# pkuyzy/ESC-GNN

Measured on AMD Instinct MI355X. Metric: graphs/sec + edges-aggregated/sec, NestedGIN_eff h=3 bs=128 @1/2/4/8 GPU, higher is better.
Workload: dtype f32; 1 GPU; count_cycle-shaped random regular graphs (n in 10/15/20/30), target=triangles, NestedGIN_eff h=3 layers=4 hidden=256, bs=128 per GPU (configs[1]); global_batch=128, parallelism=dp1 graph-sharded, rccl_ranks=1, ranks=1

## Files before the change

esc-gnn_amd/csrc/common.h:

```cpp
#pragma once
#include <hip/hip_runtime.h>
#include <hip/hip_ext.h>
#include <stdint.h>
#include <stdio.h>
#include <stdarg.h>

#include "../../include/escgnn_hip.h"

namespace esc {

constexpr int WAVE = 64;

#ifndef ESC_NODE_PRIO
#define ESC_NODE_PRIO 2
#endif
#define ESC_PRIO() __builtin_amdgcn_s_setprio(ESC_NODE_PRIO)

void set_error(const char* fmt, ...);

#define ESC_REQUIRE(cond, ...)                    \
  do {                                            \
    if (!(cond)) {                                \
      esc::set_error(__VA_ARGS__);                \
      return ESC_EINVAL;                          \
// ... 9 lines not shown
    }                                                                       \
  } while (0)

inline bool aligned16(const void* p) { return (reinterpret_cast<uintptr_t>(p) & 15) == 0; }
inline int64_t cdiv(int64_t a, int64_t b) { return (a + b - 1) / b; }

bool prof_slot(int kind, hipEvent_t* start, hipEvent_t* stop);
unsigned long long* prof_span_next(int kind);
#define ESC_SPAN_WGS 2048
#define ESC_SPAN_WAVES 8192
#define ESC_SPAN_STRIDE (ESC_SPAN_WGS + ESC_SPAN_WAVES)
bool trace_launch();

void arm_launch_event(hipEvent_t ev);
hipEvent_t take_launch_event();

template <typename... KArgs, typename... Args>
inline void launch(int kind, void (*kernel)(KArgs...), dim3 grid, dim3 block, size_t lds, hipStream_t s,
                   Args... args) {
  hipEvent_t a = nullptr, b = nullptr;
  hipEvent_t done = take_launch_event();
  if (done != nullptr) {
    hipStreamCaptureStatus cap = hipStreamCaptureStatusNone;
    if (hipStreamIsCapturing(s, &cap) != hipSuccess || cap != hipStreamCaptureStatusNone) { arm_launch_event(done); done = nullptr; }
  }
  if (prof_slot(kind, &a, &b)) {
    hipExtLaunchKernelGGL(kernel, grid, block, (unsigned)lds, s, a, b, 0, static_cast<KArgs>(args)...);
    if (done != nullptr) (void)hipEventRecord(done, s);
  } else if (done != nullptr) {
    hipExtLaunchKernelGGL(kernel, grid, block, (unsigned)lds, s, nullptr, done, 0, static_cast<KArgs>(args)...);
// ... 43 lines not shown
int gemm_lds_floor();
void set_gemm_lds_floor(int bytes);
int edge_lds_floor();
int node_lds_floor();
void set_node_lds_floor(int bytes);
void set_edge_lds_floor(int bytes);
int norm_rowblock_cap();
void set_norm_rowblock_cap(int v);
bool bn_bwd_one_launch();
void set_bn_bwd_one_launch(int on);
bool bn_bwd_fold();
void set_bn_bwd_fold(int on);
bool last_block_finalize();
void set_last_block_finalize(int on);
void set_linear_knob(int knob, int value);

__device__ __forceinline__ void store_agent(float2* p, float2 v) {
  const unsigned long long bits = ((unsigned long long)__float_as_uint(v.y) << 32) | __float_as_uint(v.x);
  __hip_atomic_store(reinterpret_cast<unsigned long long*>(p), bits, __ATOMIC_RELAXED, __HIP_MEMORY_SCOPE_AGENT);
}

__device__ __forceinline__ bool grid_last_block(unsigned* counter, unsigned nblocks) {
  __shared__ unsigned s_ticket;
  __builtin_amdgcn_s_waitcnt(0x0F70);
  __syncthreads();
  if (threadIdx.x == 0) s_ticket = __hip_atomic_fetch_add(counter, 1u, __ATOMIC_RELAXED, __HIP_MEMORY_SCOPE_AGENT);
  __syncthreads();
  const bool last = s_ticket == nblocks - 1;
  if (last) {
    __builtin_amdgcn_fence(__ATOMIC_ACQUIRE, "agent");
// ... 87 lines not shown
```

esc-gnn_amd/csrc/engine.hip:

```cpp
#include "common.h"

#include <map>
#include <vector>
#include <cstdlib>

namespace esc {

struct Arena {
  float* base;
  int64_t off;
  float* take(int64_t n) {
    float* p = base ? base + off : nullptr;
    off += (n + 63) & ~63LL;
    return p;
  }
};

struct BnWs { float *mean, *invstd, *scale, *shift, *nglob, *coef; };
struct MlpWs { float *Y0, *Y1; BnWs b0, b1; float* A1 = nullptr; };

struct Layout {
  int64_t N, E, Z, H, L, C0, W;
  float *Zb, *Yz; BnWs zb0, zb1;
  float *A0, *Zemb;
// ... 81 lines not shown
  std::vector<esc_reduce_job>* jobs = nullptr;
  float** slab_cursor = nullptr;
  bool on_edge_stream = false;
  int act = 1;
  const float* l1_target = nullptr;
  int64_t l1_denom = 0;
};

struct LdsFloorGuard {
  explicit LdsFloorGuard(bool on) : on_(on && edge_lds_floor() > 0) { if (on_) set_gemm_lds_floor(edge_lds_floor()); }
  ~LdsFloorGuard() { if (on_) set_gemm_lds_floor(0); }
  bool on_;
};

static constexpr int kNodeLdsFloorBwd = 66 * 1024;
struct NodeFloorGuard {
  explicit NodeFloorGuard(int bytes) : on_(bytes > 0) { if (on_) set_node_lds_floor(bytes); }
  ~NodeFloorGuard() { if (on_) set_node_lds_floor(0); }
  bool on_;
};

static int linear_backward(const Ctx& c, const float* dY, int64_t ld_dy, const float* X, int64_t ld_x, const float* sc,
                           const float* sh, const esc_linear_t& lin, int64_t M, float* dX, int64_t ld_dx, int accumulate) {
  const LdsFloorGuard cap(c.on_edge_stream);
  const int64_t N = lin.out_dim, K = lin.in_dim;
  if (c.jobs == nullptr)
    return esc_linear_bwd_both(dY, ld_dy, X, ld_x, sc, sh, lin.w, K, M, N, K, dX, ld_dx, accumulate, lin.dw, K, lin.db,
                               c.y.slabs, c.s);
  float* slabs = *c.slab_cursor;
  *c.slab_cursor += (esc_linear_bwd_weight_scratch(M, N, K) + 63) & ~63LL;
// ... 13 lines not shown
                              int accumulate, const esc_bn_bwd_next* next) {
  const LdsFloorGuard cap(c.on_edge_stream);
  const int64_t N = lin.out_dim, K = lin.in_dim;
  if (c.jobs == nullptr)
    return esc_linear_bwd_both_bn(dOut, ld_dout, &f, X, ld_x, sc, sh, lin.w, K, M, N, K, dX, ld_dx, accumulate, lin.dw, K, lin.db, c.y.slabs,
                                  nullptr, next, c.s);
  float* slabs = *c.slab_cursor;
  *c.slab_cursor += (esc_linear_bwd_weight_scratch(M, N, K) + 63) & ~63LL;
  c.jobs->emplace_back();
  return esc_linear_bwd_both_bn(dOut, ld_dout, &f, X, ld_x, sc, sh, lin.w, K, M, N, K, dX, ld_dx, accumulate, lin.dw, K, lin.db, slabs,
                                &c.jobs->back(), next, c.s);
}

struct EdgeStream {
  hipStream_t stream = nullptr;
  hipEvent_t z_ready = nullptr, joined = nullptr, lin1_fork = nullptr, lin1_rest = nullptr, e_ready[ESC_MAX_LAYERS] = {}, de_ready[ESC_MAX_LAYERS] = {},
             agg_done[ESC_MAX_LAYERS] = {};
  bool ok = false;
};
static int g_use_edge_stream = 1;
static int current_device() {
  int dev = 0;
  (void)hipGetDevice(&dev);
  return dev;
}
static EdgeStream& edge_stream() {
  static thread_local std::map<int, EdgeStream> per_device;
  static thread_local EdgeStream off;
  if (!g_use_edge_stream) return off;
  EdgeStream& es = per_device[current_device()];
  if (!es.ok && es.stream == nullptr) {
    int least = 0, greatest = 0;
    (void)hipDeviceGetStreamPriorityRange(&least, &greatest);
    bool good = hipStreamCreateWithPriority(&es.stream, hipStreamNonBlocking, least) == hipSuccess;
    good = good && hipEventCreateWithFlags(&es.z_ready, hipEventDisableTiming) == hipSuccess;
    good = good && hipEventCreateWithFlags(&es.joined, hipEventDisableTiming) == hipSuccess;
    good = good && hipEventCreateWithFlags(&es.lin1_fork, hipEventDisableTiming) == hipSuccess;
    good = good && hipEventCreateWithFlags(&es.lin1_rest, hipEventDisableTiming) == hipSuccess;
    for (int l = 0; l < ESC_MAX_LAYERS; ++l) {
      good = good && hipEventCreateWithFlags(&es.e_ready[l], hipEventDisableTiming) == hipSuccess;
      good = good && hipEventCreateWithFlags(&es.de_ready[l], hipEventDisableTiming) == hipSuccess;
      good = good && hipEventCreateWithFlags(&es.agg_done[l], hipEventDisableTiming) == hipSuccess;
    }
    es.ok = good;
  }
  return es;
}
static int64_t g_two_stream_min_edges = 12000;
static EdgeStream& edge_stream_for(int64_t edges) {
  static thread_local EdgeStream off;
  return edges >= g_two_stream_min_edges ? edge_stream() : off;
}
static int chain(hipEvent_t ev, hipStream_t src, hipStream_t waiter) {
  if (hipEventRecord(ev, src) != hipSuccess || hipStreamWaitEvent(waiter, ev, 0) != hipSuccess) {
    set_error("esc_engine: stream event failed");
    return ESC_ELAUNCH;
  }
  return ESC_OK;
}

static int g_plain_events = 0;
struct ArmedEvent {
  ArmedEvent(hipEvent_t ev, bool on) : on_(on && !g_plain_events) { if (on_) arm_launch_event(ev); }
  ~ArmedEvent() { if (on_) (void)take_launch_event(); }
  bool on_;
};
static int chain_armed(hipEvent_t ev, const ArmedEvent& arm, hipStream_t src, hipStream_t waiter) {
  const bool bound = arm.on_ && take_launch_event() == nullptr;
  if ((!bound && hipEventRecord(ev, src) != hipSuccess) || (waiter != nullptr && hipStreamWaitEvent(waiter, ev, 0) != hipSuccess)) {
    set_error("esc_engine: stream event failed");
    return ESC_ELAUNCH;
  }
  return ESC_OK;
}

static Ctx edge_ctx(const Ctx& c, hipStream_t edge) {
  Ctx x = c;
  x.s = edge;
  x.on_edge_stream = true;
// ... 314 lines not shown
  const Layout& y = c.y;
  const int64_t N = y.N, E = y.E, H = y.H, L = y.L, W = y.W;
  ESC_TRY(linear_backward(c, y.dpred, 1, y.Yl, H, y.bl.scale, y.bl.shift, m->lin2, N, y.dAl, H, 0));
  const bool split_lin1 = es.ok && c.jobs != nullptr && L >= 1;
  const esc_bn_bwd_fused fl = bn_fused(y.Yl, H, y.bl, 1);
  const bool fa_l = fuse_node_act(c);
  const MlpWs& wl = y.conv[L > 0 ? L - 1 : 0];
  esc_bn_bwd_next nl{y.bst_part, y.cat + L * H, W, wl.b1.mean, wl.b1.invstd, wl.b1.scale, wl.b1.shift, 1};
  auto lin1_ok = [&](int64_t col0, int64_t ncols, const esc_bn_bwd_next* nx) {
    return esc_linear_bwd_both_bn_ok(y.dAl, H, &fl, y.cat + col0, W, m->lin1.w + col0, W, N, H, ncols, y.dcat + col0, W,
                                     c.jobs ? *c.slab_cursor : y.slabs, nx) != 0;
  };
  const bool fuse_l = kBnBwdApplyInGemm && c.act == 1 && !sync_on(c) && y.bst_part != nullptr &&
                      (split_lin1 ? (lin1_ok(0, L * H, nullptr) && lin1_ok(L * H, H, nullptr)) : lin1_ok(0, W, nullptr));
  int64_t last_slots = 0;
  if (fuse_l)
    ESC_TRY(esc_bn_bwd_coef(y.Yl, H, nullptr, 0, y.dAl, H, N, H, y.bl.mean, y.bl.invstd, m->bn_lin1.gamma, m->bn_lin1.beta, 1, y.bl.coef,
                            m->bn_lin1.dgamma, m->bn_lin1.dbeta, y.bn_scratch, c.s));
  else
    ESC_TRY(bn_backward(c, y.Yl, H, nullptr, 0, y.dAl, H, N, y.bl, m->bn_lin1, y.dAl, H, y.bn_scratch));
  if (split_lin1) {
    const int64_t K0 = L * H;
    auto part = [&](void* stream, int64_t col0, int64_t ncols, float* db, const esc_bn_bwd_next* nx) -> int {
      float* slabs = *c.slab_cursor;
      *c.slab_cursor += (esc_linear_bwd_weight_scratch(N, H, ncols) + 63) & ~63LL;
      c.jobs->emplace_back();
      const bool fa = fa_l;
      if (fuse_l)
        return esc_linear_bwd_both_bn(y.dAl, H, &fl, y.cat + col0, W, fa ? y.cat_scale + col0 : nullptr, fa ? y.cat_shift + col0 : nullptr, m->lin1.w + col0, W,
                                      N, H, ncols, y.dcat + col0, W, 0, m->lin1.dw + col0, W, db, slabs, &c.jobs->back(), nx, stream);
      return esc_linear_bwd_both_deferred(y.dAl, H, y.cat + col0, W, fa ? y.cat_scale + col0 : nullptr, fa ? y.cat_shift + col0 : nullptr, m->lin1.w + col0, W, N, H, ncols,
                                          y.dcat + col0, W, 0, m->lin1.dw + col0, W, db, slabs, &c.jobs->back(), stream);
    };
    ESC_TRY(chain(es.lin1_fork, (hipStream_t)c.s, es.stream));
    {
      const LdsFloorGuard cap(true);
      ESC_TRY(part(es.stream, 0, K0, nullptr, nullptr));
    }
    if (hipEventRecord(es.lin1_rest, es.stream) != hipSuccess) { set_error("esc_engine: stream event failed"); return ESC_ELAUNCH; }
    const bool leave = fuse_l && fa_l && kBnBwdSumsFromDx && lin1_ok(K0, H, &nl) &&
                       mlp_backward_fused(c, m->conv[L - 1].nn, y.conv[L - 1], y.agg[L - 1], L == 1 ? y.C0 : H, N, y.cat + L * H, W, y.dcat + L * H, W,
                                          y.dagg, L == 1 ? y.C0 : H, true);
    ESC_TRY(part(c.s, K0, H, m->lin1.db, leave ? &nl : nullptr));
    if (leave) last_slots = cdiv(N, esc_linear_bwd_bn_block_rows(N, H, H));
  } else if (fuse_l) {
    ESC_TRY(linear_backward_bn(c, y.dAl, H, fl, y.cat, W, fa_l ? y.cat_scale : nullptr, fa_l ? y.cat_shift : nullptr, m->lin1, N, y.dcat, W, 0, nullptr));
  } else {
    ESC_TRY(linear_backward(c, y.dAl, H, y.cat, W, fa_l ? y.cat_scale : nullptr, fa_l ? y.cat_shift : nullptr, m->lin1, N, y.dcat, W, 0));
  }
  Ctx ce = es.ok ? edge_ctx(c, es.stream) : c;
  std::vector<esc_reduce_job> edge_jobs;
  edge_jobs.reserve(ESC_MAX_REDUCE_JOBS);
  if (es.ok && c.jobs) ce.jobs = &edge_jobs;
  std::vector<esc_sum_job> eps_jobs;
// ... 45 lines not shown
      ESC_TRY(esc_slab_reduce_jobs(edge_jobs.data(), (int)edge_jobs.size(), es.stream));
      edge_jobs.clear();
    }
  }
  ESC_TRY(mlp_backward(c, m->xemb, y.xemb, b->x, y.C0, N, y.cat, W, y.dcat, W, nullptr, 0, fuse_node_act(c)));
  Ctx ct = ce;
  ct.on_edge_stream = false;
  ESC_TRY(bn_backward(ce, y.Yz, H, nullptr, 0, y.dZemb, H, E, y.zb1, m->zbn1, y.dZemb, H, ce.y.bn_scratch));
  ESC_TRY(linear_backward(ct, y.dZemb, H, y.A0, H, nullptr, nullptr, m->zlin, E, y.dAz, H, 0));
  ESC_TRY(bn_backward(ce, y.Zb, H, nullptr, 0, y.dAz, H, E, y.zb0, m->zbn0, y.dAz, H, ce.y.bn_scratch));
  ESC_TRY(esc_bag_bwd_table_rows(y.dAz, H, H, b->col_ptr, b->col_row, b->col_val, b->col_col, y.Z, m->z_rows, E,
                                 1, m->dz_table, y.bag_scratch, ce.s));
  mark(PH_NODE_BWD_DONE, c.s);
  mark(PH_EDGE_BWD_DONE, ce.s);
  if (!eps_jobs.empty()) ESC_TRY(esc_reduce_sum_jobs(eps_jobs.data(), (int)eps_jobs.size(), c.s));
  if (c.jobs && !c.jobs->empty()) ESC_TRY(esc_slab_reduce_jobs(c.jobs->data(), (int)c.jobs->size(), c.s));
  if (es.ok) {
    if (hipEventRecord(es.joined, es.stream) != hipSuccess) { set_error("esc_engine: stream event failed"); return ESC_ELAUNCH; }
    Pending local;
    Pending& p = defer ? *defer : local;
    p.open = true; p.join = true; p.stream = (hipStream_t)c.s;
    p.edge_jobs.swap(edge_jobs);
    if (!defer) return finish_pending(p);
  }
  return ESC_OK;
}

static Layout plan_layout_zinc(const esc_zinc_gin_t* m, int64_t N, int64_t E, int64_t Z, int64_t G, float* base, bool train) {
  Layout y{};
  Arena a{base, 0};
// ... 518 lines not shown

}

using namespace esc;

extern "C" {

int esc_engine_set_two_stream_min_edges(int64_t edges) {
  g_two_stream_min_edges = edges < 0 ? 0 : edges;
  return ESC_OK;
}

int esc_engine_set_side_stream(int on) {
  g_use_edge_stream = (on & 2) != 0;
  g_plain_events = (on & 64) != 0;
  return ESC_OK;
}

int esc_engine_phase_times(double* out, int skip) {
  PhaseRing& p = phases();
  for (int i = 0; i < 6; ++i) out[i] = 0.0;
  if (!p.on || p.steps < 2) return 0;
  const int first = p.steps > PhaseRing::RING ? p.steps - PhaseRing::RING + 1 : 0;
  int n = 0;
  for (int sidx = first + skip; sidx < p.steps; ++sidx) {
    hipEvent_t* e = p.ev[sidx % PhaseRing::RING];
    bool ok = true;
    for (int k = 0; k < PH_COUNT; ++k) ok = ok && e[k] != nullptr;
    if (!ok) continue;
    float t[6] = {};
// ... 220 lines not shown
```

esc-gnn_amd/csrc/gemm_dma.h:

```cpp
#pragma once
#include "common.h"

namespace esc {
namespace dma {

typedef float f32x16 __attribute__((ext_vector_type(16)));
typedef int i32x4 __attribute__((ext_vector_type(4)));
using lds_void = __attribute__((address_space(3))) void;

__device__ __forceinline__ i32x4 make_rsrc(const void* p, unsigned bytes) {
  const uint64_t a = reinterpret_cast<uint64_t>(p);
  i32x4 r;
  r[0] = (int)(uint32_t)a; r[1] = (int)(uint32_t)((a >> 32) & 0xffffu); r[2] = (int)bytes; r[3] = 0x00020000;
  return r;
}
__device__ __forceinline__ unsigned lds_addr(const float* p) {
  return (unsigned)(uintptr_t)(lds_void*)const_cast<float*>(p);
}
__device__ __forceinline__ void dma16(i32x4 r, unsigned dst, int voff, int soff) {
  unsigned keep;
  asm volatile(
      "s_mov_b32 %0, m0\n\ts_mov_b32 m0, %3\n\ts_nop 4\n\tbuffer_load_dwordx4 %1, %2, %4 offen lds\n\ts_mov_b32 m0, %0"
      : "=&s"(keep)
      : "v"(voff), "s"(r), "s"(dst), "s"(soff)
// ... 688 lines not shown
template <int BM, int BN, int BK, int WM, int WN, int STAGES, int LW, bool A_RM, bool B_RM, int PRO, bool STATS, bool DB, bool INIT = false>
inline hipError_t launch_gemm(GArgs g, size_t lds_floor, hipStream_t s, int kind = ESC_K_LINEAR) {
  using C_ = Cfg<BM, BN, BK, WM, WN, STAGES, LW, A_RM, B_RM, PRO, STATS, DB>;
  auto kern = gemm_kernel<BM, BN, BK, WM, WN, STAGES, LW, A_RM, B_RM, PRO, STATS, DB, INIT>;
  if (BM < 128 && gemm_lds_floor() == 0 && (size_t)node_lds_floor() > lds_floor) lds_floor = (size_t)node_lds_floor();
  const size_t lds = C_::LDS_BYTES > lds_floor ? C_::LDS_BYTES : lds_floor;
  static size_t raised_to = 64 * 1024;
  hipError_t e = raise_lds(kern, lds, raised_to);
  if (e != hipSuccess) return e;
  finish_args<BM, BN>(g);
  const unsigned nwg = (unsigned)(g.ntile_m * g.ntile_n * splits_of(g));
  esc::launch(BM >= 128 && kind == ESC_K_LINEAR ? ESC_K_GEMM_EDGE : kind, kern, dim3(nwg), dim3(C_::NTHR), lds, s, g);
  return hipSuccess;
}

template <int BM, int BN, int BK, int WM, int WN, int STAGES, int LW, bool PRO, bool BNB = false, bool BSTAT = false>
inline hipError_t launch_dual(DualArgs a, size_t lds_floor, hipStream_t s, int kind = ESC_K_LINEAR, hipStream_t s_dw = nullptr) {
  using CX = Cfg<BM, BN, BK, WM, WN, STAGES, LW, false, true, (BNB ? 4 : 0) | (BSTAT ? 8 : 0), false, false>;
  using CW = Cfg<BM, BN, BK, WM, WN, STAGES, LW, true, true, (PRO ? 2 : 0) | (BNB ? 4 : 0), false, true>;
  auto kern = gemm_dual_kernel<BM, BN, BK, WM, WN, STAGES, LW, PRO, BNB, BSTAT>;
  const size_t lds_x = CX::LDS_BYTES + (size_t)CX::bnb_lds_floats(a.dx.R) * 4;
  size_t lds = lds_x > CW::LDS_BYTES ? lds_x : CW::LDS_BYTES;
  if (BM < 128 && gemm_lds_floor() == 0 && (size_t)node_lds_floor() > lds_floor) lds_floor = (size_t)node_lds_floor();
  if (lds_floor > lds) lds = lds_floor;
  static size_t raised_to = 64 * 1024;
  hipError_t e = raise_lds(kern, lds, raised_to);
  if (e != hipSuccess) return e;
  finish_args<BM, BN>(a.dx);
  finish_args<BM, BN>(a.dw);
  a.n_dx = a.dx.ntile_m * a.dx.ntile_n;
  a.b0 = 0;
  const unsigned n_dw = (unsigned)(a.dw.ntile_m * a.dw.ntile_n * splits_of(a.dw));
  const int k = BM >= 128 && kind == ESC_K_LINEAR ? ESC_K_GEMM_EDGE : kind;
  if (s_dw != nullptr && s_dw != s && a.n_dx > 0 && n_dw > 0) {
    esc::launch(k, kern, dim3((unsigned)a.n_dx), dim3(CX::NTHR), lds, s, a);
    a.b0 = a.n_dx;
    esc::launch(k, kern, dim3(n_dw), dim3(CX::NTHR), lds, s_dw, a);
    return hipSuccess;
  }
  esc::launch(k, kern, dim3((unsigned)a.n_dx + n_dw), dim3(CX::NTHR), lds, s, a);
  return hipSuccess;
}

}
}
```

esc-gnn_amd/csrc/linear_mfma.hip:

```cpp
#include "common.h"
#include <cstdlib>
#include "linear_plan.h"
#include "gemm_tile.h"
#include "gemm_dma.h"
#include "linear_small.h"
#include "linear_narrow.h"

namespace esc {

using plan::Flags;
using plan::Op;
using plan::Plan;

static plan::PlanKnobs g_plan;
void set_linear_knob(int knob, int value) {
  if (knob == 11) g_plan.use_dma = value;
  else g_plan.knob[knob] = value;
}
static const plan::PlanKnobs& knobs() {
  static const bool env_read = [] {
    if (getenv("ESC_BIG_MIN_WGS")) g_plan.big_min_wgs = atoll(getenv("ESC_BIG_MIN_WGS"));
    if (getenv("ESC_TILE160")) g_plan.tile160 = atoi(getenv("ESC_TILE160"));
    if (getenv("ESC_TILE160_MIN_WGS")) g_plan.tile160_min_wgs = atoll(getenv("ESC_TILE160_MIN_WGS"));
    return true;
  }();
  (void)env_read;
  return g_plan;
}

using DmaBnCfg = dma::Cfg<64, 64, 32, 2, 2, 2, 2, false, true, 4, false, false>;
static_assert(DmaBnCfg::BNB_MAXK == BNB_MAX_N && DmaBnCfg::PRO_MAXK == PRO_MAX_K, "linear_plan.h and gemm_dma.h disagree on the LDS-resident vectors");
static_assert(plan::R01_TILE[1].bm == 64 && plan::R01_TILE[1].bn == 64 && plan::R01_TILE[1].bk == 32 && plan::R01_TILE[1].kw == 1, "tile 1 is the default tile");

// ... 489 lines not shown
                                 const float* in_shift, const float* W, int64_t ld_w, int64_t M, int64_t N, int64_t K,
                                 float* dX, int64_t ld_dx, int accumulate, float* dW, int64_t ld_dw, float* db,
                                 float* slabs, esc_reduce_job* job, void* stream) {
  ESC_REQUIRE(job, "esc_linear_bwd_both_deferred: null job");
  return both_impl(dY, ld_dy, X, ld_x, in_scale, in_shift, W, ld_w, M, N, K, dX, ld_dx, accumulate, dW, ld_dw, db, slabs,
                   job, stream);
}

static Plan plan_both_bn(const float* dOut, int64_t ld_dout, const esc_bn_bwd_fused* b, const float* X, int64_t ld_x, const float* W,
                         int64_t ld_w, int64_t M, int64_t N, int64_t K, const float* dX, int64_t ld_dx, const float* slabs,
                         const esc_bn_bwd_next* n) {
  plan::BnOps bo{};
  plan::NextOps no{};
  if (b) bo = plan::BnOps{b->x, b->ld_x, b->mean, b->invstd, b->scale, b->shift, b->coef, b->relu};
  if (n) no = plan::NextOps{n->partial, n->x, n->ld_x, n->mean, n->invstd, n->scale, n->shift, n->relu};
  return plan::plan_both_bn(knobs(), Op{dOut, ld_dout}, b ? &bo : nullptr, Op{X, ld_x}, Op{W, ld_w}, Op{dX, ld_dx}, slabs, n ? &no : nullptr,
                            M, N, K);
}

int esc_linear_bwd_both_bn_ok(const float* dOut, int64_t ld_dout, const esc_bn_bwd_fused* bn, const float* X, int64_t ld_x,
                              const float* W, int64_t ld_w, int64_t M, int64_t N, int64_t K, const float* dX, int64_t ld_dx,
                              const float* slabs, const esc_bn_bwd_next* next) {
  return plan_both_bn(dOut, ld_dout, bn, X, ld_x, W, ld_w, M, N, K, dX, ld_dx, slabs, next).ok ? 1 : 0;
}

int64_t esc_linear_bwd_bn_block_rows(int64_t M, int64_t N, int64_t K) { return plan::bwd_bn_block_rows(M, N, K); }

int esc_linear_bwd_both_bn(const float* dOut, int64_t ld_dout, const esc_bn_bwd_fused* bn, const float* X, int64_t ld_x,
                           const float* in_scale, const float* in_shift, const float* W, int64_t ld_w, int64_t M,
                           int64_t N, int64_t K, float* dX, int64_t ld_dx, int accumulate, float* dW, int64_t ld_dw,
                           float* db, float* slabs, esc_reduce_job* defer, const esc_bn_bwd_next* next, void* stream) {
// ... 7 lines not shown
                       : BnbDev{};
  if (p.family == plan::F_SMALL_BN) {
    const int act = bd.relu == 2 ? 2 : 1;
    launch_wgrad_small(dOut, ld_dout, X, ld_x, in_scale, in_shift, M, N, K, slabs, p, bd, act, s);
    ESC_CHECK_LAUNCH("esc_linear_bwd_both_bn.small");
    if (dX != nullptr) {
      ESC_TRY_(launch_smalln_dx(dOut, ld_dout, W, ld_w, M, N, K, dX, ld_dx, accumulate, bd, act, "esc_linear_bwd_both_bn", s));
      ESC_CHECK_LAUNCH("esc_linear_bwd_both_bn.smalln");
    }
    return reduce_slabs(p, slabs, N, K, dW, ld_dw, db, defer, stream);
  }
  dma::DualArgs a{};
  dma_fill_dx(a.dx, dOut, ld_dout, W, ld_w, M, N, K, dX, ld_dx, accumulate);
  dma_fill_dw(a.dw, dOut, ld_dout, X, ld_x, in_scale, in_shift, M, N, K, slabs, p);
  a.dx.bnb = bd; a.dw.bnb = bd;
  if (next)
    a.dx.bst = BnStatDev{reinterpret_cast<float2*>(next->partial), next->x, (int)next->ld_x, next->mean, next->invstd, next->scale, next->shift, next->relu};
  hipError_t e;
#define ESC_T64_2STAGE 64, 64, 32, 2, 2, 2, 2
  if (p.family == plan::F_DMA128_BN) {
    if (next) e = in_scale ? dma::launch_dual<ESC_T128, true, true, true>(a, 0, s) : dma::launch_dual<ESC_T128, false, true, true>(a, 0, s);
    else      e = in_scale ? dma::launch_dual<ESC_T128, true, true, false>(a, 0, s) : dma::launch_dual<ESC_T128, false, true, false>(a, 0, s);
  } else {
    if (bn == nullptr) e = in_scale ? dma::launch_dual<ESC_T64, true, false, true>(a, 0, s) : dma::launch_dual<ESC_T64, false, false, true>(a, 0, s);
    else if (next)     e = in_scale ? dma::launch_dual<ESC_T64_2STAGE, true, true, true>(a, 0, s) : dma::launch_dual<ESC_T64_2STAGE, false, true, true>(a, 0, s);
    else               e = in_scale ? dma::launch_dual<ESC_T64_2STAGE, true, true, false>(a, 0, s) : dma::launch_dual<ESC_T64_2STAGE, false, true, false>(a, 0, s);
  }
#undef ESC_T64_2STAGE
  if (dma_check(e, "esc_linear_bwd_both_bn") != hipSuccess) return ESC_ELAUNCH;
  return reduce_slabs(p, slabs, N, K, dW, ld_dw, db, defer, stream);
}

}
```

esc-gnn_amd/csrc/linear_plan.h:

```cpp
#pragma once
#include <cstddef>
#include <cstdint>

namespace esc {

namespace small {
constexpr int SMALL_MAX = 16;
constexpr int ROWS_FWD = 32;
constexpr int SMALLN_DX_MAX_N = ((160 * 1024 / 4) / (32 + SMALL_MAX) - 4) & ~3;
constexpr int ROWS_WGRAD = 32;
}

constexpr int NARROW_N = 4, NARROW_K = 256;
constexpr int NARROW_ROWS = 32;
constexpr int NARROW_DX_N = 16;
constexpr int64_t PRO_MAX_K = 1280;
constexpr int64_t BNB_MAX_N = 640;
constexpr int64_t FUSE_FINALIZE_MAX_ROWS = 4096;
constexpr int64_t EDGE_ROWS = 8192;

namespace plan {

inline int64_t cdiv(int64_t a, int64_t b) { return (a + b - 1) / b; }
inline bool aligned16(const void* p) { return (reinterpret_cast<uintptr_t>(p) & 15) == 0; }

enum { KNOB_FWD_BIG = 0, KNOB_FWD_SMALL = 1, KNOB_DX_BIG = 2, KNOB_DX_SMALL = 3, KNOB_DW_TILE = 4,
       KNOB_DW_BLOCKS = 5, KNOB_DW_MIN_ROWS = 6, KNOB_DUAL_SMALL = 7, KNOB_COUNT = 8 };
struct PlanKnobs {
  int knob[KNOB_COUNT] = {1, 4, 1, 4, 4, 512, 128, 2};
  int use_dma = 15;
  int tile160 = 0;
  int64_t tile160_min_wgs = 150;
  int64_t big_min_wgs = 1LL << 62;
};

struct Tile { int bm, bn, wm, wn, bk, kw; };
constexpr int R01_TILES = 11;
constexpr Tile R01_TILE[R01_TILES] = {
    {128, 128, 2, 2, 32, 1}, {64, 64, 2, 2, 32, 1}, {128, 32, 4, 1, 32, 1}, {128, 64, 2, 2, 32, 1}, {64, 64, 2, 2, 64, 1},
    {32, 64, 1, 2, 32, 1},   {32, 32, 1, 1, 32, 1}, {64, 32, 2, 1, 32, 1},  {32, 32, 1, 1, 64, 4},  {32, 32, 1, 1, 128, 4},
    {64, 32, 2, 1, 64, 2}};
inline int r01_tile_id(int id, bool db) { return (id < 0 || id >= R01_TILES || (db && id >= 8)) ? 1 : id; }

enum Family {
  F_NONE = 0,
  F_NARROW, F_SMALLK, F_DMA64X32, F_DMA64, F_DMA128, F_DMA128X64, F_DMA160, F_R01,
  F_R01_ROWSTATS,
  F_R01_BN,
// ... 13 lines not shown
  return (f >= 0 && f < F_COUNT) ? names[f] : "?";
}

enum BnAfter { BN_NONE = 0, BN_FROM_ROWS , BN_FROM_PARTIALS ,
               BN_IN_KERNEL };

struct Plan {
  Family family = F_NONE;
  bool ok = false;
  int tile = 1;
  int bm = 0, bn = 0;
  int block_rows = 32;
  BnAfter bn_after = BN_NONE;
  int splits = 0, per_split = 0;
  int64_t slab_floats = 0;
};

struct Op { const void* p; int64_t ld; };
struct Flags {
  bool pro = false;
  bool pro_aligned = true;
  bool pro_paired = true;
  bool col_stats = false;
  bool c_init = false;
  bool fold = false;
  bool bn = false;
  bool last_block_finalize = false;
};

inline bool vec_ok(Op a) { return aligned16(a.p) && a.ld % 4 == 0; }
// ... 172 lines not shown
inline Plan plan_both_bn(const PlanKnobs& k, Op dOut, const BnOps* bn, Op X, Op W, Op dX, const void* slabs, const NextOps* next,
                         int64_t M, int64_t N, int64_t K) {
  Plan p;
  if (!dOut.p || !X.p || !W.p || !slabs || M <= 1 || N <= 0 || K <= 0 || (bn == nullptr && next == nullptr)) return p;
  const bool big = bwd_big(M, N, K);
  if (edge_sized(M) && !(big && bn != nullptr && N <= BNB_MAX_N)) return p;
  if (bn != nullptr && !bn_ops_ok(*bn, M, N)) return p;
  p.block_rows = (int)bwd_bn_block_rows(M, N, K);
  if (bn != nullptr && (k.use_dma & 4) && K <= small::SMALL_MAX && N > small::SMALL_MAX && N % 4 == 0 && N <= small::SMALLN_DX_MAX_N) {
    if (next != nullptr || !vec_ok(dOut) || dOut.ld < N || X.ld < K || W.ld < K || (dX.p != nullptr && dX.ld < K)) return p;
    return with_splits(with_family(p, F_SMALL_BN, 0, 256), cdiv(M, small::ROWS_WGRAD), small::ROWS_WGRAD, N, K);
  }
  if (dX.p == nullptr || N > BNB_MAX_N) return p;
  if (!dma_bwd_ok(k, dOut, &X, &W, &dX, slabs, M, N, K)) return p;
  if (next != nullptr && !next_ops_ok(*next, dX, K)) return p;
  return dma_wgrad_splits(big ? with_family(p, F_DMA128_BN, 128, 128) : with_family(p, F_DMA64_BN, 64, 64), M, N, K);
}

static_assert(NARROW_ROWS == small::ROWS_WGRAD, "one promise covers both 32-row plans");
inline int64_t bwd_weight_scratch(int64_t M, int64_t N, int64_t K) {
  const bool fine = (K <= small::SMALL_MAX) != (N <= small::SMALL_MAX) || (N <= NARROW_N && K <= NARROW_K);
  return (cdiv(M, fine ? small::ROWS_WGRAD : 128) + 1) * (N * K + N);
}

}
}
```

esc-gnn_amd/csrc/norm.hip:

```cpp
#include "common.h"
#include "norm_plan.h"

#include <type_traits>

namespace esc {

static inline bool act_code_ok(int act) { return act >= 0 && act <= 2; }

__device__ __forceinline__ float act_fwd(float v, int act) {
  if (act == 1) return fmaxf(v, 0.f);
  if (act == 2) return v > 0.f ? v : expm1f(v);
  return v;
}
__device__ __forceinline__ float act_grad_from_out(float y, int act) {
  if (act == 1) return y > 0.f ? 1.f : 0.f;
  if (act == 2) return y > 0.f ? 1.f : y + 1.f;
  return 1.f;
}
__device__ __forceinline__ float pre_act_fwd(float x, float mu, float is, float ga, float be) {
  const float sc = ga * is;
  return fmaf(x, sc, be - mu * sc);
}
__device__ __forceinline__ float pre_act_bwd(float x, float xh, float mu, float is, float ga, float be, int act) {
  return act == 2 ? fmaf(xh, ga, be) : pre_act_fwd(x, mu, is, ga, be);
// ... 842 lines not shown
              reinterpret_cast<float2*>(coef), (int)C, n_total);
  ESC_CHECK_LAUNCH("esc_bn_sync_coef");
  return ESC_OK;
}

int esc_bn_eval_coef(const float* running_mean, const float* running_var, const float* gamma, const float* beta,
                     float eps, int64_t C, float* scale, float* shift, void* stream) {
  ESC_REQUIRE(running_mean && running_var && scale && shift && C > 0, "esc_bn_eval_coef: bad argument");
  esc::launch(ESC_K_NORM, bn_eval_coef_kernel, dim3((unsigned)cdiv(C, 256)), dim3(256), 0, (hipStream_t)stream,
              running_mean, running_var, gamma, beta, eps, (int)C, scale, shift);
  ESC_CHECK_LAUNCH("esc_bn_eval_coef");
  return ESC_OK;
}

static int bn_bwd_reduce(const BwdArgs& a, const norm::Plan& p, int64_t divisor, float* dgamma, float* dbeta, float2* partial, float2* coef,
                         hipStream_t s) {
  const bool fused = p.reduce == norm::R_FUSED;
  if (p.reduce == norm::R_SCALAR) {
    esc::launch(ESC_K_NORM, bn_bwd_partial_kernel, dim(p.grid[0]), dim3(256), 0, s, a.X, a.ld_x, a.Y, a.ld_y, a.dY, a.ld_dy, (int)a.M, (int)a.C, a.mean,
                a.invstd, a.relu, a.gamma, a.beta, partial);
  } else {
    unsigned* tk = fused ? tickets((int)p.grid[0].x) : nullptr;
    ESC_REQUIRE(!fused || tk != nullptr, "esc_bn_bwd: no ticket counters");
    launch_bwd_partial_v4(a, p.grid[0], partial, tk, dgamma, dbeta, coef, s);
  }
  if (!fused) {
    ESC_CHECK_LAUNCH("esc_bn_bwd.partial");
    launch_bwd_finalize(partial, divisor, a.C, p.slots, dgamma, dbeta, coef, s);
  }
  ESC_CHECK_LAUNCH("esc_bn_bwd.finalize");
  return ESC_OK;
}

static int bn_bwd_apply_impl(const BwdArgs& a, norm::Apply form, Grid g, const float2* coef, float* dX, int64_t ld_dx, hipStream_t s) {
  if (form == norm::A_ROWS) launch_bwd_rows(a, g, false, coef, dX, ld_dx, 0, nullptr, nullptr, s);
  else with_act(a.relu, a.Y != nullptr, [&](auto act, auto has_y) {
    constexpr int A = decltype(act)::value;
    constexpr bool H = decltype(has_y)::value;
    esc::launch(ESC_K_NORM, form == norm::A_FLAT4 ? bn_bwd_apply_kernel<4, A, H> : bn_bwd_apply_kernel<1, A, H>, dim(g), dim3(256), 0, s, a.X, a.ld_x,
                a.Y, a.ld_y, a.dY, a.ld_dy, a.M, (int)a.C, a.mean, a.invstd, a.gamma, a.beta, coef, dX, ld_dx);
  });
  ESC_CHECK_LAUNCH("esc_bn_bwd.apply");
// ... 82 lines not shown
  ESC_REQUIRE(M > 0 && C > 0 && ld_x >= C && ld_dy >= C && (!Y || ld_y >= C) && M < (1LL << 31), "esc_bn_bwd_sums: bad sizes");
  ESC_REQUIRE(act_code_ok(relu), "esc_bn_bwd_sums: relu must be 0 (none), 1 (ReLU) or 2 (ELU), got %d", relu);
  const BwdArgs a{X, ld_x, Y, ld_y, dY, ld_dy, M, C, mean, invstd, gamma, beta, relu};
  const norm::Plan p = norm::plan_bwd_reduce(knobs(), ops_of(a, nullptr, 0, scratch, nullptr, nullptr, nullptr), M, C, false, false);
  return bn_bwd_reduce(a, p, 1, dgamma, dbeta, (float2*)scratch, (float2*)sums, (hipStream_t)stream);
}

int esc_bn_bwd_coef(const float* X, int64_t ld_x, const float* Y, int64_t ld_y, const float* dY, int64_t ld_dy, int64_t M,
                    int64_t C, const float* mean, const float* invstd, const float* gamma, const float* beta, int relu,
                    float* coef, float* dgamma, float* dbeta, float* scratch, void* stream) {
  ESC_REQUIRE(X && dY && coef && mean && invstd && scratch, "esc_bn_bwd_coef: null pointer");
  ESC_REQUIRE(M > 0 && C > 0 && ld_x >= C && ld_dy >= C && (!Y || ld_y >= C) && M < (1LL << 31), "esc_bn_bwd_coef: bad sizes");
  ESC_REQUIRE(act_code_ok(relu), "esc_bn_bwd_coef: relu must be 0 (none), 1 (ReLU) or 2 (ELU), got %d", relu);
  const BwdArgs a{X, ld_x, Y, ld_y, dY, ld_dy, M, C, mean, invstd, gamma, beta, relu};
  const norm::Plan p = norm::plan_bwd_reduce(knobs(), ops_of(a, nullptr, 0, scratch, nullptr, nullptr, nullptr), M, C, true, true);
  return bn_bwd_reduce(a, p, M, dgamma, dbeta, (float2*)scratch, (float2*)coef, (hipStream_t)stream);
}

int esc_bn_bwd_coef_from_partials(const float* partial, int64_t slots, int64_t M, int64_t C, float* coef, float* dgamma,
                                  float* dbeta, void* stream) {
  ESC_REQUIRE(partial && coef && slots > 0 && M > 0 && C > 0 && M < (1LL << 31) && slots < (1LL << 31), "esc_bn_bwd_coef_from_partials: bad arguments");
  launch_bwd_finalize(reinterpret_cast<const float2*>(partial), M, C, slots, dgamma, dbeta, reinterpret_cast<float2*>(coef), (hipStream_t)stream);
  ESC_CHECK_LAUNCH("esc_bn_bwd_coef_from_partials");
  return ESC_OK;
}

int esc_bn_bwd_apply(const float* X, int64_t ld_x, const float* Y, int64_t ld_y, const float* dY,
                     int64_t ld_dy, int64_t M, int64_t C, const float* mean, const float* invstd,
                     const float* gamma, const float* beta, int relu, const float* coef, float* dX,
                     int64_t ld_dx, void* stream) {
  ESC_REQUIRE(X && dY && dX && mean && invstd && coef, "esc_bn_bwd_apply: null pointer");
// ... 9 lines not shown
```

esc-gnn_amd/csrc/runtime.hip:

```cpp
#include "common.h"
#include "linear_plan.h"
#include <algorithm>
#include <cstdlib>

#include <mutex>
#include <vector>

namespace esc {

static thread_local char g_err[512] = "";

void set_error(const char* fmt, ...) {
  va_list ap;
  va_start(ap, fmt);
  vsnprintf(g_err, sizeof(g_err), fmt, ap);
  va_end(ap);
}

struct ProfState {
  bool on = false;
  std::vector<hipEvent_t> start, stop;
  size_t used = 0;
};
static ProfState g_prof[ESC_K_COUNT];
// ... 39 lines not shown
void set_last_block_finalize(int on) { g_last_block = on != 0; }

static thread_local int g_gemm_lds_floor = 0;
int gemm_lds_floor() { return g_gemm_lds_floor; }
void set_gemm_lds_floor(int bytes) { g_gemm_lds_floor = bytes < 0 ? 0 : (bytes > 160 * 1024 ? 160 * 1024 : bytes); }
static int g_edge_lds_floor = 52 * 1024;
int edge_lds_floor() { return g_edge_lds_floor; }
static thread_local int g_node_lds_floor = 0;
int node_lds_floor() { return g_node_lds_floor; }
void set_node_lds_floor(int bytes) { g_node_lds_floor = bytes < 0 ? 0 : (bytes > 160 * 1024 ? 160 * 1024 : bytes); }
void set_edge_lds_floor(int bytes) { g_edge_lds_floor = bytes < 0 ? 0 : bytes; }

static thread_local hipEvent_t g_launch_event = nullptr;
void arm_launch_event(hipEvent_t ev) { g_launch_event = ev; }
hipEvent_t take_launch_event() { hipEvent_t ev = g_launch_event; g_launch_event = nullptr; return ev; }

static const bool g_trace_launch = getenv("ESC_TRACE_LAUNCH") != nullptr && atoi(getenv("ESC_TRACE_LAUNCH")) != 0;
bool trace_launch() { return g_trace_launch; }
static int g_bn_bwd_one = getenv("ESC_BN_BWD_ONE") ? atoi(getenv("ESC_BN_BWD_ONE")) : 0;
bool bn_bwd_one_launch() { return g_bn_bwd_one != 0; }
void set_bn_bwd_one_launch(int on) { g_bn_bwd_one = on != 0; }
static int g_bn_bwd_fold = 0;
bool bn_bwd_fold() { return g_bn_bwd_fold != 0; }
void set_bn_bwd_fold(int on) { g_bn_bwd_fold = on != 0; }
static int g_norm_rowblock_cap = 256;
int norm_rowblock_cap() { return g_norm_rowblock_cap; }
void set_norm_rowblock_cap(int v) { g_norm_rowblock_cap = v < 1 ? 1 : (v > 512 ? 512 : v); }

unsigned* tickets(int n) {
  int dev = 0;
// ... 9 lines not shown
  unsigned* out = g_tickets[dev] + g_ticket_pos[dev];
  g_ticket_pos[dev] += n;
  return out;
}

}

extern "C" {

int esc_tune_set(int knob, int value) {
  if (knob == 8) { esc::set_last_block_finalize(value); return ESC_OK; }
  if (knob == 9) { esc::set_norm_rowblock_cap(value); return ESC_OK; }
  if (knob == 12) { esc::set_bn_bwd_fold(value); return ESC_OK; }
  if (knob == 13) { esc::set_bn_bwd_one_launch(value); return ESC_OK; }
  if (knob == 10) { esc::set_edge_lds_floor(value); return ESC_OK; }
  ESC_REQUIRE(knob == 11 || (knob >= 0 && knob < esc::plan::KNOB_COUNT), "esc_tune_set: unknown knob %d", knob);
  esc::set_linear_knob(knob, value);
  return ESC_OK;
}

int esc_abi_version(void) { return ESC_ABI_VERSION; }
const char* esc_last_error(void) { return esc::g_err; }

int esc_prof_enable(int kind, int on) {
  ESC_REQUIRE(kind >= 0 && kind < ESC_K_COUNT, "esc_prof_enable: bad kind %d", kind);
  std::lock_guard<std::mutex> lk(esc::g_prof_mu);
  esc::g_prof[kind].on = on != 0;
  return ESC_OK;
}

int esc_prof_reset(int kind) {
// ... 77 lines not shown
```

Baseline: 134,700 graphs/s.

## Split readout dual GEMM into separate dX and dW launches with event signalling

```diff
diff --git a/esc-gnn_amd/csrc/common.h b/esc-gnn_amd/csrc/common.h
--- a/esc-gnn_amd/csrc/common.h
+++ b/esc-gnn_amd/csrc/common.h
@@ -47,6 +47,9 @@
 
 void arm_launch_event(hipEvent_t ev);
 hipEvent_t take_launch_event();
+void arm_last_launch_event(hipEvent_t ev);
+void next_launch_is_last();
+hipEvent_t take_last_launch_event();
 
 template <typename... KArgs, typename... Args>
 inline void launch(int kind, void (*kernel)(KArgs...), dim3 grid, dim3 block, size_t lds, hipStream_t s,
@@ -120,6 +123,9 @@
 bool last_block_finalize();
 void set_last_block_finalize(int on);
 void set_linear_knob(int knob, int value);
+struct DualSplit { hipEvent_t dx_done = nullptr, dw_done = nullptr; int dx_lds = 0; };
+void request_dual_split(const DualSplit& r);
+bool take_dual_split();
 
 __device__ __forceinline__ void store_agent(float2* p, float2 v) {
   const unsigned long long bits = ((unsigned long long)__float_as_uint(v.y) << 32) | __float_as_uint(v.x);
diff --git a/esc-gnn_amd/csrc/engine.hip b/esc-gnn_amd/csrc/engine.hip
--- a/esc-gnn_amd/csrc/engine.hip
+++ b/esc-gnn_amd/csrc/engine.hip
@@ -119,6 +119,9 @@
 };
 
 static constexpr int kNodeLdsFloorBwd = 66 * 1024;
+static constexpr int kReadoutDxLds = 84 * 1024;
+static_assert(2 * kReadoutDxLds > 160 * 1024 && kReadoutDxLds + kNodeLdsFloorBwd <= 160 * 1024, "one readout dX tile and one node tile per CU");
+static int g_readout_one_launch = 0;
 struct NodeFloorGuard {
   explicit NodeFloorGuard(int bytes) : on_(bytes > 0) { if (on_) set_node_lds_floor(bytes); }
   ~NodeFloorGuard() { if (on_) set_node_lds_floor(0); }
@@ -162,7 +165,7 @@
 
 struct EdgeStream {
   hipStream_t stream = nullptr;
-  hipEvent_t z_ready = nullptr, joined = nullptr, lin1_fork = nullptr, lin1_rest = nullptr, e_ready[ESC_MAX_LAYERS] = {}, de_ready[ESC_MAX_LAYERS] = {},
+  hipEvent_t z_ready = nullptr, joined = nullptr, lin1_fork = nullptr, lin1_rest = nullptr, lin1_dw = nullptr, e_ready[ESC_MAX_LAYERS] = {}, de_ready[ESC_MAX_LAYERS] = {},
              agg_done[ESC_MAX_LAYERS] = {};
   bool ok = false;
 };
@@ -185,6 +188,7 @@
     good = good && hipEventCreateWithFlags(&es.joined, hipEventDisableTiming) == hipSuccess;
     good = good && hipEventCreateWithFlags(&es.lin1_fork, hipEventDisableTiming) == hipSuccess;
     good = good && hipEventCreateWithFlags(&es.lin1_rest, hipEventDisableTiming) == hipSuccess;
+    good = good && hipEventCreateWithFlags(&es.lin1_dw, hipEventDisableTiming) == hipSuccess;
     for (int l = 0; l < ESC_MAX_LAYERS; ++l) {
       good = good && hipEventCreateWithFlags(&es.e_ready[l], hipEventDisableTiming) == hipSuccess;
       good = good && hipEventCreateWithFlags(&es.de_ready[l], hipEventDisableTiming) == hipSuccess;
@@ -211,6 +215,12 @@
 struct ArmedEvent {
   ArmedEvent(hipEvent_t ev, bool on) : on_(on && !g_plain_events) { if (on_) arm_launch_event(ev); }
   ~ArmedEvent() { if (on_) (void)take_launch_event(); }
+  bool on_;
+};
+struct ArmedLastEvent {
+  ArmedLastEvent(hipEvent_t ev, bool on) : on_(on && !g_plain_events) { if (on_) arm_last_launch_event(ev); }
+  ~ArmedLastEvent() { if (on_) (void)take_last_launch_event(); }
+  bool bound() const { return on_ && take_last_launch_event() == nullptr; }
   bool on_;
 };
 static int chain_armed(hipEvent_t ev, const ArmedEvent& arm, hipStream_t src, hipStream_t waiter) {
@@ -555,10 +565,14 @@
   const bool fuse_l = kBnBwdApplyInGemm && c.act == 1 && !sync_on(c) && y.bst_part != nullptr &&
                       (split_lin1 ? (lin1_ok(0, L * H, nullptr) && lin1_ok(L * H, H, nullptr)) : lin1_ok(0, W, nullptr));
   int64_t last_slots = 0;
-  if (fuse_l)
+  bool k0_split = false;
+  bool fork_bound = false;
+  if (fuse_l) {
+    const ArmedLastEvent arm(es.lin1_fork, split_lin1);
     ESC_TRY(esc_bn_bwd_coef(y.Yl, H, nullptr, 0, y.dAl, H, N, H, y.bl.mean, y.bl.invstd, m->bn_lin1.gamma, m->bn_lin1.beta, 1, y.bl.coef,
                             m->bn_lin1.dgamma, m->bn_lin1.dbeta, y.bn_scratch, c.s));
-  else
+    fork_bound = arm.bound();
+  } else
     ESC_TRY(bn_backward(c, y.Yl, H, nullptr, 0, y.dAl, H, N, y.bl, m->bn_lin1, y.dAl, H, y.bn_scratch));
   if (split_lin1) {
     const int64_t K0 = L * H;
@@ -573,12 +587,19 @@
       return esc_linear_bwd_both_deferred(y.dAl, H, y.cat + col0, W, fa ? y.cat_scale + col0 : nullptr, fa ? y.cat_shift + col0 : nullptr, m->lin1.w + col0, W, N, H, ncols,
                                           y.dcat + col0, W, 0, m->lin1.dw + col0, W, db, slabs, &c.jobs->back(), stream);
     };
-    ESC_TRY(chain(es.lin1_fork, (hipStream_t)c.s, es.stream));
+    if ((!fork_bound && hipEventRecord(es.lin1_fork, (hipStream_t)c.s) != hipSuccess) || hipStreamWaitEvent(es.stream, es.lin1_fork, 0) != hipSuccess) {
+      set_error("esc_engine: stream event failed");
+      return ESC_ELAUNCH;
+    }
     {
       const LdsFloorGuard cap(true);
-      ESC_TRY(part(es.stream, 0, K0, nullptr, nullptr));
-    }
-    if (hipEventRecord(es.lin1_rest, es.stream) != hipSuccess) { set_error("esc_engine: stream event failed"); return ESC_ELAUNCH; }
+      const bool ask = fuse_l && !g_readout_one_launch && !g_plain_events;
+      if (ask) request_dual_split(DualSplit{es.lin1_rest, es.lin1_dw, kReadoutDxLds});
+      const int rc = part(es.stream, 0, K0, nullptr, nullptr);
+      k0_split = !take_dual_split() && ask;
+      ESC_TRY(rc);
+    }
+    if (!k0_split && hipEventRecord(es.lin1_rest, es.stream) != hipSuccess) { set_error("esc_engine: stream event failed"); return ESC_ELAUNCH; }
     const bool leave = fuse_l && fa_l && kBnBwdSumsFromDx && lin1_ok(K0, H, &nl) &&
                        mlp_backward_fused(c, m->conv[L - 1].nn, y.conv[L - 1], y.agg[L - 1], L == 1 ? y.C0 : H, N, y.cat + L * H, W, y.dcat + L * H, W,
                                           y.dagg, L == 1 ? y.C0 : H, true);
@@ -654,6 +675,7 @@
   mark(PH_NODE_BWD_DONE, c.s);
   mark(PH_EDGE_BWD_DONE, ce.s);
   if (!eps_jobs.empty()) ESC_TRY(esc_reduce_sum_jobs(eps_jobs.data(), (int)eps_jobs.size(), c.s));
+  if (k0_split && hipStreamWaitEvent((hipStream_t)c.s, es.lin1_dw, 0) != hipSuccess) { set_error("esc_engine: stream event failed"); return ESC_ELAUNCH; }
   if (c.jobs && !c.jobs->empty()) ESC_TRY(esc_slab_reduce_jobs(c.jobs->data(), (int)c.jobs->size(), c.s));
   if (es.ok) {
     if (hipEventRecord(es.joined, es.stream) != hipSuccess) { set_error("esc_engine: stream event failed"); return ESC_ELAUNCH; }
@@ -1202,6 +1224,7 @@
 int esc_engine_set_side_stream(int on) {
   g_use_edge_stream = (on & 2) != 0;
   g_plain_events = (on & 64) != 0;
+  g_readout_one_launch = (on & 128) != 0;
   return ESC_OK;
 }
 
diff --git a/esc-gnn_amd/csrc/gemm_dma.h b/esc-gnn_amd/csrc/gemm_dma.h
--- a/esc-gnn_amd/csrc/gemm_dma.h
+++ b/esc-gnn_amd/csrc/gemm_dma.h
@@ -726,8 +726,16 @@
   return hipSuccess;
 }
 
+struct DualEvents { bool split = false; hipEvent_t dx_done = nullptr, dw_done = nullptr; size_t dx_lds = 0; };
+template <typename K>
+inline hipError_t launch_signalling(hipEvent_t ev, int kind, K kern, unsigned nwg, unsigned nthr, size_t lds, hipStream_t s, const DualArgs& a) {
+  if (ev != nullptr) arm_launch_event(ev);
+  esc::launch(kind, kern, dim3(nwg), dim3(nthr), lds, s, a);
+  return (ev != nullptr && take_launch_event() != nullptr) ? hipEventRecord(ev, s) : hipSuccess;
+}
 template <int BM, int BN, int BK, int WM, int WN, int STAGES, int LW, bool PRO, bool BNB = false, bool BSTAT = false>
-inline hipError_t launch_dual(DualArgs a, size_t lds_floor, hipStream_t s, int kind = ESC_K_LINEAR, hipStream_t s_dw = nullptr) {
+inline hipError_t launch_dual(DualArgs a, size_t lds_floor, hipStream_t s, int kind = ESC_K_LINEAR, hipStream_t s_dw = nullptr,
+                              DualEvents ev = DualEvents{}) {
   using CX = Cfg<BM, BN, BK, WM, WN, STAGES, LW, false, true, (BNB ? 4 : 0) | (BSTAT ? 8 : 0), false, false>;
   using CW = Cfg<BM, BN, BK, WM, WN, STAGES, LW, true, true, (PRO ? 2 : 0) | (BNB ? 4 : 0), false, true>;
   auto kern = gemm_dual_kernel<BM, BN, BK, WM, WN, STAGES, LW, PRO, BNB, BSTAT>;
@@ -750,9 +758,19 @@
     esc::launch(k, kern, dim3(n_dw), dim3(CX::NTHR), lds, s_dw, a);
     return hipSuccess;
   }
-  esc::launch(k, kern, dim3((unsigned)a.n_dx + n_dw), dim3(CX::NTHR), lds, s, a);
-  return hipSuccess;
-}
-
-}
-}
+  if (ev.split && a.n_dx > 0 && n_dw > 0) {
+    const size_t lds_dx = ev.dx_lds > lds ? ev.dx_lds : lds;
+    e = raise_lds(kern, lds_dx, raised_to);
+    if (e != hipSuccess) return e;
+    e = launch_signalling(ev.dx_done, k, kern, (unsigned)a.n_dx, CX::NTHR, lds_dx, s, a);
+    if (e != hipSuccess) return e;
+    a.b0 = a.n_dx;
+    return launch_signalling(ev.dw_done, k, kern, n_dw, CX::NTHR, lds, s, a);
+  }
+  e = launch_signalling(ev.dw_done, k, kern, (unsigned)a.n_dx + n_dw, CX::NTHR, lds, s, a);
+  if (e != hipSuccess || ev.dx_done == nullptr) return e;
+  return hipEventRecord(ev.dx_done, s);
+}
+
+}
+}
diff --git a/esc-gnn_amd/csrc/linear_mfma.hip b/esc-gnn_amd/csrc/linear_mfma.hip
--- a/esc-gnn_amd/csrc/linear_mfma.hip
+++ b/esc-gnn_amd/csrc/linear_mfma.hip
@@ -15,8 +15,13 @@
 static plan::PlanKnobs g_plan;
 void set_linear_knob(int knob, int value) {
   if (knob == 11) g_plan.use_dma = value;
+  else if (knob == 14) g_plan.dual_split = value;
   else g_plan.knob[knob] = value;
 }
+static thread_local DualSplit t_dual_split;
+static thread_local bool t_dual_split_on = false;
+void request_dual_split(const DualSplit& r) { t_dual_split = r; t_dual_split_on = true; }
+bool take_dual_split() { const bool pending = t_dual_split_on; t_dual_split_on = false; t_dual_split = DualSplit{}; return pending; }
 static const plan::PlanKnobs& knobs() {
   static const bool env_read = [] {
     if (getenv("ESC_BIG_MIN_WGS")) g_plan.big_min_wgs = atoll(getenv("ESC_BIG_MIN_WGS"));
@@ -536,7 +541,9 @@
   plan::NextOps no{};
   if (b) bo = plan::BnOps{b->x, b->ld_x, b->mean, b->invstd, b->scale, b->shift, b->coef, b->relu};
   if (n) no = plan::NextOps{n->partial, n->x, n->ld_x, n->mean, n->invstd, n->scale, n->shift, n->relu};
-  return plan::plan_both_bn(knobs(), Op{dOut, ld_dout}, b ? &bo : nullptr, Op{X, ld_x}, Op{W, ld_w}, Op{dX, ld_dx}, slabs, n ? &no : nullptr,
+  plan::PlanKnobs k = knobs();
+  if (t_dual_split_on) k.dual_split = t_dual_split.dx_lds > 1 ? t_dual_split.dx_lds : 1;
+  return plan::plan_both_bn(k, Op{dOut, ld_dout}, b ? &bo : nullptr, Op{X, ld_x}, Op{W, ld_w}, Op{dX, ld_dx}, slabs, n ? &no : nullptr,
                             M, N, K);
 }
 
@@ -574,17 +581,21 @@
   dma_fill_dx(a.dx, dOut, ld_dout, W, ld_w, M, N, K, dX, ld_dx, accumulate);
   dma_fill_dw(a.dw, dOut, ld_dout, X, ld_x, in_scale, in_shift, M, N, K, slabs, p);
   a.dx.bnb = bd; a.dw.bnb = bd;
+  dma::DualEvents ev{};
+  ev.split = p.launches == 2;
+  ev.dx_lds = (size_t)p.dx_lds;
+  if (ev.split && t_dual_split_on) { ev.dx_done = t_dual_split.dx_done; ev.dw_done = t_dual_split.dw_done; (void)take_dual_split(); }
   if (next)
     a.dx.bst = BnStatDev{reinterpret_cast<float2*>(next->partial), next->x, (int)next->ld_x, next->mean, next->invstd, next->scale, next->shift, next->relu};
   hipError_t e;
 #define ESC_T64_2STAGE 64, 64, 32, 2, 2, 2, 2
   if (p.family == plan::F_DMA128_BN) {
-    if (next) e = in_scale ? dma::launch_dual<ESC_T128, true, true, true>(a, 0, s) : dma::launch_dual<ESC_T128, false, true, true>(a, 0, s);
-    else      e = in_scale ? dma::launch_dual<ESC_T128, true, true, false>(a, 0, s) : dma::launch_dual<ESC_T128, false, true, false>(a, 0, s);
+    if (next) e = in_scale ? dma::launch_dual<ESC_T128, true, true, true>(a, 0, s, ESC_K_LINEAR, nullptr, ev) : dma::launch_dual<ESC_T128, false, true, true>(a, 0, s, ESC_K_LINEAR, nullptr, ev);
+    else      e = in_scale ? dma::launch_dual<ESC_T128, true, true, false>(a, 0, s, ESC_K_LINEAR, nullptr, ev) : dma::launch_dual<ESC_T128, false, true, false>(a, 0, s, ESC_K_LINEAR, nullptr, ev);
   } else {
-    if (bn == nullptr) e = in_scale ? dma::launch_dual<ESC_T64, true, false, true>(a, 0, s) : dma::launch_dual<ESC_T64, false, false, true>(a, 0, s);
-    else if (next)     e = in_scale ? dma::launch_dual<ESC_T64_2STAGE, true, true, true>(a, 0, s) : dma::launch_dual<ESC_T64_2STAGE, false, true, true>(a, 0, s);
-    else               e = in_scale ? dma::launch_dual<ESC_T64_2STAGE, true, true, false>(a, 0, s) : dma::launch_dual<ESC_T64_2STAGE, false, true, false>(a, 0, s);
+    if (bn == nullptr) e = in_scale ? dma::launch_dual<ESC_T64, true, false, true>(a, 0, s, ESC_K_LINEAR, nullptr, ev) : dma::launch_dual<ESC_T64, false, false, true>(a, 0, s, ESC_K_LINEAR, nullptr, ev);
+    else if (next)     e = in_scale ? dma::launch_dual<ESC_T64_2STAGE, true, true, true>(a, 0, s, ESC_K_LINEAR, nullptr, ev) : dma::launch_dual<ESC_T64_2STAGE, false, true, true>(a, 0, s, ESC_K_LINEAR, nullptr, ev);
+    else               e = in_scale ? dma::launch_dual<ESC_T64_2STAGE, true, true, false>(a, 0, s, ESC_K_LINEAR, nullptr, ev) : dma::launch_dual<ESC_T64_2STAGE, false, true, false>(a, 0, s, ESC_K_LINEAR, nullptr, ev);
   }
 #undef ESC_T64_2STAGE
   if (dma_check(e, "esc_linear_bwd_both_bn") != hipSuccess) return ESC_ELAUNCH;
diff --git a/esc-gnn_amd/csrc/linear_plan.h b/esc-gnn_amd/csrc/linear_plan.h
--- a/esc-gnn_amd/csrc/linear_plan.h
+++ b/esc-gnn_amd/csrc/linear_plan.h
@@ -17,6 +17,7 @@
 constexpr int64_t PRO_MAX_K = 1280;
 constexpr int64_t BNB_MAX_N = 640;
 constexpr int64_t FUSE_FINALIZE_MAX_ROWS = 4096;
+constexpr int LDS_BYTES = 160 * 1024;
 constexpr int64_t EDGE_ROWS = 8192;
 
 namespace plan {
@@ -32,6 +33,7 @@
   int tile160 = 0;
   int64_t tile160_min_wgs = 150;
   int64_t big_min_wgs = 1LL << 62;
+  int dual_split = 0;
 };
 
 struct Tile { int bm, bn, wm, wn, bk, kw; };
@@ -75,6 +77,8 @@
   BnAfter bn_after = BN_NONE;
   int splits = 0, per_split = 0;
   int64_t slab_floats = 0;
+  int launches = 1;
+  int dx_lds = 0;
 };
 
 struct Op { const void* p; int64_t ld; };
@@ -277,6 +281,7 @@
   if (dX.p == nullptr || N > BNB_MAX_N) return p;
   if (!dma_bwd_ok(k, dOut, &X, &W, &dX, slabs, M, N, K)) return p;
   if (next != nullptr && !next_ops_ok(*next, dX, K)) return p;
+  if (k.dual_split > 0) { p.launches = 2; p.dx_lds = k.dual_split > 1 ? (k.dual_split < LDS_BYTES ? k.dual_split : LDS_BYTES) : 0; }
   return dma_wgrad_splits(big ? with_family(p, F_DMA128_BN, 128, 128) : with_family(p, F_DMA64_BN, 64, 64), M, N, K);
 }
 
diff --git a/esc-gnn_amd/csrc/norm.hip b/esc-gnn_amd/csrc/norm.hip
--- a/esc-gnn_amd/csrc/norm.hip
+++ b/esc-gnn_amd/csrc/norm.hip
@@ -880,8 +880,9 @@
 }
 
 static int bn_bwd_reduce(const BwdArgs& a, const norm::Plan& p, int64_t divisor, float* dgamma, float* dbeta, float2* partial, float2* coef,
-                         hipStream_t s) {
+                         hipStream_t s, bool ends_call = false) {
   const bool fused = p.reduce == norm::R_FUSED;
+  if (fused && ends_call) next_launch_is_last();
   if (p.reduce == norm::R_SCALAR) {
     esc::launch(ESC_K_NORM, bn_bwd_partial_kernel, dim(p.grid[0]), dim3(256), 0, s, a.X, a.ld_x, a.Y, a.ld_y, a.dY, a.ld_dy, (int)a.M, (int)a.C, a.mean,
                 a.invstd, a.relu, a.gamma, a.beta, partial);
@@ -892,6 +893,7 @@
   }
   if (!fused) {
     ESC_CHECK_LAUNCH("esc_bn_bwd.partial");
+    if (ends_call) next_launch_is_last();
     launch_bwd_finalize(partial, divisor, a.C, p.slots, dgamma, dbeta, coef, s);
   }
   ESC_CHECK_LAUNCH("esc_bn_bwd.finalize");
@@ -1004,7 +1006,7 @@
   ESC_REQUIRE(act_code_ok(relu), "esc_bn_bwd_coef: relu must be 0 (none), 1 (ReLU) or 2 (ELU), got %d", relu);
   const BwdArgs a{X, ld_x, Y, ld_y, dY, ld_dy, M, C, mean, invstd, gamma, beta, relu};
   const norm::Plan p = norm::plan_bwd_reduce(knobs(), ops_of(a, nullptr, 0, scratch, nullptr, nullptr, nullptr), M, C, true, true);
-  return bn_bwd_reduce(a, p, M, dgamma, dbeta, (float2*)scratch, (float2*)coef, (hipStream_t)stream);
+  return bn_bwd_reduce(a, p, M, dgamma, dbeta, (float2*)scratch, (float2*)coef, (hipStream_t)stream, true);
 }
 
 int esc_bn_bwd_coef_from_partials(const float* partial, int64_t slots, int64_t M, int64_t C, float* coef, float* dgamma,
diff --git a/esc-gnn_amd/csrc/runtime.hip b/esc-gnn_amd/csrc/runtime.hip
--- a/esc-gnn_amd/csrc/runtime.hip
+++ b/esc-gnn_amd/csrc/runtime.hip
@@ -77,6 +77,16 @@
 static thread_local hipEvent_t g_launch_event = nullptr;
 void arm_launch_event(hipEvent_t ev) { g_launch_event = ev; }
 hipEvent_t take_launch_event() { hipEvent_t ev = g_launch_event; g_launch_event = nullptr; return ev; }
+static thread_local hipEvent_t g_last_launch_event = nullptr;
+void arm_last_launch_event(hipEvent_t ev) { g_last_launch_event = ev; }
+void next_launch_is_last() {
+  if (g_last_launch_event != nullptr) { g_launch_event = g_last_launch_event; g_last_launch_event = nullptr; }
+}
+hipEvent_t take_last_launch_event() {
+  hipEvent_t ev = g_last_launch_event != nullptr ? g_last_launch_event : g_launch_event;
+  g_last_launch_event = nullptr; g_launch_event = nullptr;
+  return ev;
+}
 
 static const bool g_trace_launch = getenv("ESC_TRACE_LAUNCH") != nullptr && atoi(getenv("ESC_TRACE_LAUNCH")) != 0;
 bool trace_launch() { return g_trace_launch; }
@@ -116,7 +126,7 @@
   if (knob == 12) { esc::set_bn_bwd_fold(value); return ESC_OK; }
   if (knob == 13) { esc::set_bn_bwd_one_launch(value); return ESC_OK; }
   if (knob == 10) { esc::set_edge_lds_floor(value); return ESC_OK; }
-  ESC_REQUIRE(knob == 11 || (knob >= 0 && knob < esc::plan::KNOB_COUNT), "esc_tune_set: unknown knob %d", knob);
+  ESC_REQUIRE(knob == 11 || knob == 14 || (knob >= 0 && knob < esc::plan::KNOB_COUNT), "esc_tune_set: unknown knob %d", knob);
   esc::set_linear_knob(knob, value);
   return ESC_OK;
 }
```

Result: faster. 136,900 graphs/s, median of 6 (+1.7%).
